# kaiidams/Kokoro-Align

Hardware: AMD Instinct MI355X
Metric: aligned audio-frames/sec (whole node), 50k x 5k lattice (higher is better)
Workload: dtype f32; 1 GPU; cfg2: T=50000 x V=64 log-probs, S=5000 phonemes (L=10001), beam_size=1000, max_move=4; batch of 8192 independent lattices per GPU per step, as 4 launches of 2048 on 4 streams; lattices_per_gpu=8192, parallelism=lattice-sharded x1, kernel_form=auto, backtrace=auto, streams_per_gpu=4

## Files before the change

kokoro-align_amd/csrc/ka_wave_backtrace.hpp:

```cpp
#pragma once
#include "ka_device.hpp"

namespace ka {

constexpr int kRcMinWaves = 8;

constexpr int kBtChunk = 16;
constexpr int kBtReach = 3 * 2 * kBtChunk;
constexpr int kBtBlocks = kBtChunk / 2;
constexpr int kBtRegs = kBtChunk * kBtBlocks / 64;
constexpr int kBtGroupsPerReg = 16 / kBtBlocks;
static_assert(16 * kBtBlocks >= kBtReach + 31, "window too narrow for the prefetch distance");

__device__ __forceinline__ int bt_window(int p_entry)
{
    const int lo = p_entry - kBtReach;
    return (lo > 0 ? lo : 0) >> 4;
}
__device__ __forceinline__ uint32_t bt_lane_offset(int w0, int lane)
{
    const int j = lane % kBtBlocks, fr = (lane / kBtBlocks) & 3, g = lane / (4 * kBtBlocks);
    return (uint32_t)g * 1024u + (uint32_t)((w0 + j) & 63) * 16u + (uint32_t)fr * 4u;
}
__device__ __forceinline__ void bt_load_guarded(uint32_t (&r)[kBtRegs], const char *chunk_base, int n, int w0, int lane)
{
    const int fr = (lane / kBtBlocks) & 3, g = lane / (4 * kBtBlocks);
    const uint32_t voff = bt_lane_offset(w0, lane);
#pragma unroll
    for (int v = 0; v < kBtRegs; ++v) {
        const int f = 4 * (v * kBtGroupsPerReg + g) + fr;
        r[v] = f < n ? *(gcu32_t)(chunk_base + (size_t)v * kBtGroupsPerReg * 1024 + voff) : 0u;
    }
}
__device__ __forceinline__ void bt_load_async(uint32_t (&r)[kBtRegs], const char *chunk_base , int w0, int lane)
{
    const uint32_t voff = bt_lane_offset(w0, lane);
#pragma unroll
    for (int v = 0; v < kBtRegs; ++v)
        asm volatile("global_load_dword %0, %1, %2" : "=&v"(r[v]) : "v"(voff), "s"(chunk_base + (size_t)v * kBtGroupsPerReg * 1024) : "memory");
}
template <int N>
__device__ __forceinline__ void bt_wait(uint32_t (&r)[2])
{
    asm volatile("s_waitcnt vmcnt(%2)" : "+v"(r[0]), "+v"(r[1]) : "i"(N) : "memory");
}
template <bool FULL>
__device__ __forceinline__ void bt_walk(const uint32_t (&r)[kBtRegs], int n, int w0, int &p, int &pathv)
{
    int q = p - 16 * w0;
    const int base = 16 * w0;
    uint32_t rr[kBtRegs];
#pragma unroll
    for (int i = 0; i < kBtRegs; ++i) rr[i] = blank_to_uniform(r[i]);
#pragma unroll
    for (int f = kBtChunk - 1; f >= 0; --f) {
        if (FULL || f < n) {
            const int grp = f >> 2;
            const int lane_base = ((grp % kBtGroupsPerReg) * 4 + (f & 3)) * kBtBlocks;
            const uint32_t w = (uint32_t)__builtin_amdgcn_readlane((int)rr[grp / kBtGroupsPerReg], (q >> 4) | lane_base);
            asm("v_writelane_b32 %0, %1, %2" : "+v"(pathv) : "s"(q), "i"(f));
            q -= bp_decode(w >> ((q * 2) & 31));
        }
    }
    pathv += base;
    p = q + base;
}

__global__ __launch_bounds__(64) void backtrace_w16_kernel(const Lattice *__restrict__ lats, const int32_t *meta, int only_flagged)
{
    const Lattice &d = lats[blockIdx.x];
    const int lane = threadIdx.x;
    if (only_flagged && !(__builtin_amdgcn_readfirstlane(meta[4 * (size_t)d.idx + 2]) & kFlagExact)) return;
    int p = __builtin_amdgcn_readfirstlane(meta[4 * (size_t)d.idx + 1]);
    if (p < 0) return;
    const char *bp = reinterpret_cast<const char *>(d.bp);
    gi32_t path = (gi32_t)d.path;
    const int T = __builtin_amdgcn_readfirstlane(d.T);
    uint32_t cur[kBtRegs], nxt[kBtRegs];
    int t0 = ((T - 1) / kBtChunk) * kBtChunk;
    int w = bt_window(p + 3 * kBtChunk);
    {
        const int n = T - t0;
        bt_load_guarded(cur, bp + (size_t)t0 * 256, n, w, lane);
        const int t1 = t0 > 0 ? t0 - kBtChunk : 0;
        const int wn = bt_window(p);
        bt_load_async(nxt, bp + (size_t)t1 * 256, wn, lane);
        int pathv = 0;
        bt_walk<false>(cur, n, w, p, pathv);
        if (lane < n) path[t0 + lane] = pathv;
        bt_wait<1>(nxt);
#pragma unroll
        for (int i = 0; i < kBtRegs; ++i) cur[i] = nxt[i];
        w = wn;
    }
    while (t0 > 0) {
        t0 -= kBtChunk;
        const int t1 = t0 > 0 ? t0 - kBtChunk : 0;
        const int wn = bt_window(p);
        bt_load_async(nxt, bp + (size_t)t1 * 256, wn, lane);
        int pathv = 0;
        bt_walk<true>(cur, kBtChunk, w, p, pathv);
        if (lane < kBtChunk) path[t0 + lane] = pathv;
        bt_wait<1>(nxt);
#pragma unroll
        for (int i = 0; i < kBtRegs; ++i) cur[i] = nxt[i];
        w = wn;
    }
}

__device__ __forceinline__ uint32_t rc_blank_to_uniform(uint32_t x)
{
    const uint32_t h = (x >> 3) & 0x11111111u, l = (x >> 2) & 0x11111111u;
    return (x & 0x33333333u) | ((h | l) << 3) | (h << 2);
}
__device__ __forceinline__ uint64_t lane_field(uint32_t count, uint32_t first)
{
    uint64_t m;
    asm("s_bfm_b64 %0, %1, %2" : "=s"(m) : "s"(count), "s"(first));
    return m;
}
#define KA_RC_E0_OUT "=&s"
#define KA_RC_E0_IN "s"
#define KA_RC_GATHER "ds_bpermute_b32 %[eln], %[lab4], %[rown]\n\tv_readfirstlane_b32 %[e0n], %[rown]\n\t"
#define KA_RC_HEAD                                                                        \
    KA_RC_GATHER                                                                          \
    "v_add_f32 %[t2], %[e0], %[sl]\n\t"                                                   \
    "v_add_f32_dpp %[t4], %[sl], %[el] wave_ror:1 row_mask:0xf bank_mask:0xf\n\t"         \
    "v_add_f32_dpp %[t5], %[sb], %[el] wave_ror:1 row_mask:0xf bank_mask:0xf\n\t"         \
    "v_add_f32 %[t0], %[e0], %[sb]\n\t"                                                   \
    "v_add_f32 %[t3], %[sb], %[el]\n\t"                                                   \
    "v_add_f32 %[t7], %[sl], %[el]\n\t"                                                   \
    "v_mov_b32_dpp %[t1], %[t2] wave_ror:1 row_mask:0xf bank_mask:0xf\n\t"                \
    "v_max_f32 %[t6], %[t7], %[t3]\n\t"
#define KA_RC_VETO "v_min_f32 %[t4], %[t4], %[veto]\n\t"
#define KA_RC_MAX                                                                         \
    "v_max3_f32 %[sl], %[t6], %[t4], %[t5]\n\t"                                           \
    "s_nop 0\n\t"                                                                         \
    "v_mov_b32_dpp %[t2], %[t1] wave_ror:1 row_mask:0xf bank_mask:0xf\n\t"                \
    "v_max3_f32 %[sb], %[t0], %[t1], %[t2]\n\t"
#define KA_RC_COMBINE                                                                     \
    "s_or_b64 %[sx], %[sa], %[sb2]\n\t"                                                   \
    "v_addc_co_u32 %[w], %[sy], %[w], %[w], %[sx]\n\t"                                    \
    "s_andn2_b64 %[sc], %[sc], %[sb2]\n\t"                                                \
    "s_or_b64 %[sc], %[sc], %[sa]\n\t"                                                    \
    "v_addc_co_u32 %[w], %[sy], %[w], %[w], %[sc]\n\t"
#define KA_RC_CODES                                                                       \
    "v_cmp_eq_f32 %[sa], %[t0], %[sb]\n\t"                                                \
    "v_addc_co_u32 %[w], %[sy], %[w], %[w], %[sa]\n\t"                                    \
    "v_cmp_eq_f32 %[sa], %[t1], %[sb]\n\t"                                                \
    "v_addc_co_u32 %[w], %[sy], %[w], %[w], %[sa]\n\t"                                    \
    "v_cmp_eq_f32 %[sa], %[t7], %[sl]\n\t"                                                \
    "v_cmp_eq_f32 %[sb2], %[t3], %[sl]\n\t"                                               \
    "v_cmp_eq_f32 %[sc], %[t4], %[sl]\n\t"                                                \
    KA_RC_COMBINE
#define KA_RC_BAND                                                                        \
    "s_bitcmp1_b32 %[open], 0\n\t"                                                        \
    "s_cbranch_scc1 .Lka_rc_open_%=\n\t"                                                  \
    "v_cndmask_b32 %[sb], %[ninf], %[sb], %[mb]\n\t"                                      \
    "v_cndmask_b32 %[sl], %[ninf], %[sl], %[ml]\n"                                        \
    ".Lka_rc_open_%=:\n\t"                                                                \
    "s_waitcnt lgkmcnt(0)"
#define KA_RC_OUTS                                                                                                              \
    [sb] "+v"(sb), [sl] "+v"(sl), [w] "+v"(word), [eln] "=&v"(el_next), [e0n] KA_RC_E0_OUT(e0_next), [t0] "=&v"(t0), [t1] "=&v"(t1),   \
    [t2] "=&v"(t2), [t3] "=&v"(t3), [t4] "=&v"(t4), [t5] "=&v"(t5), [t6] "=&v"(t6), [t7] "=&v"(t7), [sa] "=&s"(sa),             \
    [sb2] "=&s"(sb2), [sc] "=&s"(sc), [sx] "=&s"(sx), [sy] "=&s"(sy)
#define KA_RC_INS                                                                                                               \
    [e0] KA_RC_E0_IN(e0), [el] "v"(el), [rown] "v"(row_next), [lab4] "v"(lab4), [zero] "v"(zero), [open] "s"(open), [mb] "s"(mask_b),   \
    [ml] "s"(mask_l), [ninf] "v"(NINF)
template <bool ZL>
__device__ __forceinline__ void rc_frame4(float &sb, float &sl, uint32_t &word, float e0, float el, float &e0_next, float &el_next,
                                          float row_next, int lab4, int zero, float veto, uint32_t open, uint64_t mask_b,
                                          uint64_t mask_l, float NINF)
{
    float t0, t1, t2, t3, t4, t5, t6, t7;
    uint64_t sa, sb2, sc, sx, sy;
    if constexpr (ZL)
        asm volatile(KA_RC_HEAD KA_RC_VETO KA_RC_MAX KA_RC_CODES KA_RC_BAND : KA_RC_OUTS : KA_RC_INS, [veto] "v"(veto) : "memory", "scc");
    else
        asm volatile(KA_RC_HEAD KA_RC_MAX KA_RC_CODES KA_RC_BAND : KA_RC_OUTS : KA_RC_INS : "memory", "scc");
}
#undef KA_RC_HEAD
#undef KA_RC_GATHER
#undef KA_RC_E0_OUT
#undef KA_RC_E0_IN
#undef KA_RC_VETO
#undef KA_RC_MAX
#undef KA_RC_CODES
#undef KA_RC_COMBINE
#undef KA_RC_BAND
#undef KA_RC_OUTS
#undef KA_RC_INS
constexpr int kRcLanes = 62;

template <bool FULL>
__device__ __forceinline__ void rc_walk_out(const uint32_t (&codes)[kCkFrames / 8], const float (&rows)[kCkFrames], int lab4, int n,
                                            int lane, int &qq, int &pathv, int &labv, float &scv)
{
    constexpr int G = kCkFrames / 8;
    static_assert(kCkFrames == 32, "one bit per frame in a 32-bit move mask");
    const int q_in = qq;
    int j = qq >> 1;
    uint32_t cw[G];
#pragma unroll
    for (int g = 0; g < G; ++g) cw[g] = (uint32_t)__builtin_amdgcn_readlane((int)codes[g], j);
    int cl = __builtin_amdgcn_readlane(lab4, j);
    int col = (qq & 1) ? cl >> 2 : 0;
    uint32_t par = (qq & 1) ? 0u : 2u;
    uint32_t mlo = 0, mhi = 0;
#pragma unroll
    for (int f = kCkFrames - 1; f >= 0; --f) {
        if (FULL || f < n) {
            const int sc = __builtin_amdgcn_readlane(__builtin_bit_cast(int, rows[f]), col);
            asm("v_writelane_b32 %0, %1, %2" : "+v"(scv) : "s"(sc), "i"(f));
            const uint32_t mv = (uint32_t)bp_decode(cw[f >> 3] >> (4 * (7 - (f & 7)) + par));
            if (mv != 0) {
                qq -= (int)mv;
                mlo |= (mv & 1u) << f;
                mhi |= (mv >> 1) << f;
                if (f > 0) {
                    par = (qq & 1) ? 0u : 2u;
                    if ((qq >> 1) != j) {
                        j = qq >> 1;
#pragma unroll
                        for (int g = 0; g <= (f - 1) >> 3; ++g) cw[g] = (uint32_t)__builtin_amdgcn_readlane((int)codes[g], j);
                        cl = __builtin_amdgcn_readlane(lab4, j);
                    }
                    col = (qq & 1) ? cl >> 2 : 0;
                }
            }
        }
    }
    const uint32_t above_lo = (mlo >> 1) >> (lane & 31), above_hi = (mhi >> 1) >> (lane & 31);
    pathv = q_in - (__builtin_popcount(above_lo) + 2 * __builtin_popcount(above_hi));
    const int l4 = __builtin_amdgcn_ds_bpermute((pathv >> 1) << 2, lab4);
    labv = (pathv & 1) ? l4 >> 2 : 0;
}

template <int M, bool ZL, bool PAR>
__device__ __forceinline__ void backtrace_rc_body(const Lattice *__restrict__ lats, const int32_t *meta, int n_lats)
{
    const int which = PAR ? __builtin_amdgcn_readfirstlane(lattice_of_chunk(lats, n_lats, (int64_t)blockIdx.x)) : (int)blockIdx.x;
    const Lattice &d = lats[which];
    const int lane = threadIdx.x;
    if (!PAR && __builtin_amdgcn_readfirstlane(d.par)) return;
    const int32_t *mt = meta + 4 * (size_t)d.idx;
    const int flags = __builtin_amdgcn_readfirstlane(mt[2]);
    if (flags & (kFlagExact | kFlagDeclined)) return;
    if (((flags & kFlagZeroLabel) != 0) != ZL) return;
    if (__builtin_amdgcn_readfirstlane(mt[0]) != kStatusOk) return;
    int p = __builtin_amdgcn_readfirstlane(mt[1]);
    if (p < 0) return;
    const uint32_t T = (uint32_t)__builtin_amdgcn_readfirstlane(d.T);
    const uint32_t L = (uint32_t)__builtin_amdgcn_readfirstlane(d.L);
    const uint32_t B = (uint32_t)__builtin_amdgcn_readfirstlane(d.beam);
    const uint32_t halfB = B >> 1;
    const uint32_t dq = L / T, dr = L % T;
    const float NINF = ninf();
    const char *lp = reinterpret_cast<const char *>(d.lp);
    const size_t ldb = (size_t)d.ld * 4;
    const uint32_t col_off = (lane < d.V ? (uint32_t)lane : 0u) * 4u;
    gci32_t labx = (gci32_t)d.labx;
    const char *ck = reinterpret_cast<const char *>(d.bp);
    const uint32_t ck_mask = (uint32_t)__builtin_amdgcn_readfirstlane((int)d.ck_mask);
    const size_t ck_pitch = (size_t)(uint32_t)__builtin_amdgcn_readfirstlane(d.ck_pitch);
    gi32_t path = (gi32_t)d.path;
    gi32_t lab_out = (gi32_t)d.lab_out;
    gf32_t sc_out = (gf32_t)d.sc_out;

    uint32_t t0 = ((T - 1) / kCkFrames) * kCkFrames;
    if constexpr (PAR) {
        const uint32_t c = (uint32_t)((int64_t)blockIdx.x - d.chunk0);
        t0 = c * kCkFrames;
        p = __builtin_amdgcn_readfirstlane(d.entry[c]);
    }
    const auto uni = [](uint64_t v) { return (uint32_t)__builtin_amdgcn_readfirstlane((int)(uint32_t)v); };
    uint32_t q0 = uni(((uint64_t)L * t0) / T), r0 = uni(((uint64_t)L * t0) % T);
    const uint32_t D32 = uni(((uint64_t)L * kCkFrames) / T), R32 = uni(((uint64_t)L * kCkFrames) % T);
    const float inv_T = 1.0f / (float)T;

    for (;;) {
        const int n = (int)(T - t0 < (uint32_t)kCkFrames ? T - t0 : (uint32_t)kCkFrames);
        const int wlo = __builtin_amdgcn_readfirstlane((p > 96 ? p - 96 : 0) & ~1);
        const int pb = wlo + 2 * lane;
        int lab4;
        asm volatile("global_load_dword %0, %1, %2" : "=v"(lab4) : "v"((uint32_t)lane * 4u), "s"(labx + (wlo >> 1)) : "memory");
        f32x2 ckv = {NINF, NINF};
        if (t0 != 0) {
            const uint32_t off = ((uint32_t)pb & ck_mask) * 4u;
            asm volatile("global_load_dwordx2 %0, %1, %2" : "=v"(ckv) : "v"(off), "s"(ck + ((size_t)(t0 / kCkFrames) - 1) * ck_pitch) : "memory");
        }
        float rows[kCkFrames];
        {
            const char *rp = lp + (size_t)t0 * ldb;
            if (n == kCkFrames) {
#pragma unroll
                for (int f = 0; f < kCkFrames; ++f) {
                    rows[f] = row_load(col_off, rp);
                    rp += ldb;
                }
            } else {
#pragma unroll
                for (int f = 0; f < kCkFrames; ++f) {
                    rows[f] = row_load(col_off, rp);
                    rp += (f + 1 < n) ? ldb : 0;
                }
            }
        }
        asm volatile("s_waitcnt vmcnt(%2)" : "+v"(lab4), "+v"(ckv) : "i"(kCkFrames) : "memory");
        const float veto = lab4 == 0 ? NINF : __builtin_inff();
        float sb, sl;
        if (t0 == 0) {
            sb = pb == 0 ? 0.0f : NINF;
            sl = NINF;
        } else {
            const uint32_t qm = r0 >= dr ? q0 - dq : q0 - dq - 1;
            const int32_t dl = (int32_t)qm - (int32_t)halfB;
            const uint32_t lo1 = (uint32_t)(dl > 0 ? dl : 0);
            const uint32_t hi1 = (L - lo1 < B) ? L : lo1 + B;
            sb = ((uint32_t)pb >= lo1 && (uint32_t)pb < hi1 && lane < kRcLanes) ? ckv.x : NINF;
            sl = ((uint32_t)pb + 1 >= lo1 && (uint32_t)pb + 1 < hi1 && lane < kRcLanes) ? ckv.y : NINF;
        }
        uint32_t codes[kCkFrames / 8] = {};
        const auto div_T = [&](uint32_t x) {
            uint32_t qe = (uint32_t)((float)x * inv_T);
            qe -= (qe * T > x) ? 1u : 0u;
            qe += (x - qe * T >= T) ? 1u : 0u;
            return qe;
        };
        const uint32_t qnum = r0 + (uint32_t)lane * dr;
        const uint32_t qa = q0 + (uint32_t)lane * dq + div_T(qnum);
        uint64_t mask_b = 0, mask_l = 0;
        const auto band_masks = [&](int f) {
            const uint32_t q = (uint32_t)__builtin_amdgcn_readlane((int)qa, f);
            const int32_t dl = (int32_t)q - (int32_t)halfB;
            const int32_t lo = dl > 0 ? dl : 0;
            const int32_t hi = (L - (uint32_t)lo < B) ? (int32_t)L : lo + (int32_t)B;
            int32_t x = lo - wlo, y = hi - wlo;
            x = x < 0 ? 0 : x;
            y = y < 0 ? 0 : y;
            asm("" : "+s"(x), "+s"(y));
            x = x > 2 * kRcLanes ? 2 * kRcLanes : x;
            y = y > 2 * kRcLanes ? 2 * kRcLanes : y;
            const uint32_t xb = (uint32_t)(x + 1) >> 1, yb = (uint32_t)(y + 1) >> 1, xl = (uint32_t)x >> 1, yl = (uint32_t)y >> 1;
            mask_b = lane_field(yb - xb, xb);
            mask_l = lane_field(yl - xl, xl);
        };
        if constexpr (M == 4) {
            bool open = false;
            if (t0 != 0 && n == kCkFrames) {
                const uint32_t q_last = (uint32_t)__builtin_amdgcn_readlane((int)qa, kCkFrames - 1);
                const int32_t dl_last = (int32_t)q_last - (int32_t)halfB;
                const uint32_t qm = r0 >= dr ? q0 - dq : q0 - dq - 1;
                const int32_t dl = (int32_t)qm - (int32_t)halfB;
                const uint32_t lo1 = (uint32_t)(dl > 0 ? dl : 0);
                const uint32_t hi1 = (L - lo1 < B) ? L : lo1 + B;
                open = wlo > 0 && dl_last <= wlo && (uint32_t)p < hi1;
            }
            const int zero = 0;
            float e0c, elc, e0n, eln;
            row_wait_n(rows[0], kCkFrames - 1);
            asm volatile("ds_bpermute_b32 %0, %2, %4\n\t"
                         "v_readfirstlane_b32 %1, %4\n\t"
                         "s_waitcnt lgkmcnt(0)"
                         : "=&v"(elc), "=&s"(e0c) : "v"(lab4), "v"(zero), "v"(rows[0]) : "memory");
            uint32_t moves = 0;
            const uint32_t open_bit = (uint32_t)__builtin_amdgcn_readfirstlane(open ? 1 : 0);
            if (open_bit) {
                sb = ckv.x;
                sl = ckv.y;
            } else {
                const uint32_t qb = q0 + (uint32_t)(lane + 1) * dq + div_T(qnum + dr);
                moves = (uint32_t)__builtin_amdgcn_ballot_w64(qa != qb) << 1 | 1u;
            }
            asm volatile("s_nop 1" : "+v"(sb), "+v"(sl));
#pragma unroll
            for (int f = 0; f < kCkFrames; ++f) {
                if ((moves >> f) & 1u) band_masks(f);
                if (f + 1 < kCkFrames) row_wait_n(rows[f + 1], kCkFrames - 2 - f);
                rc_frame4<ZL>(sb, sl, codes[f >> 3], e0c, elc, e0n, eln, rows[f + 1 < kCkFrames ? f + 1 : f], lab4, zero, veto,
                              open_bit, mask_b, mask_l, NINF);
                e0c = e0n;
                elc = eln;
            }
        } else {
            const uint32_t qb = q0 + (uint32_t)(lane + 1) * dq + div_T(qnum + dr);
            const uint32_t moves = (uint32_t)__builtin_amdgcn_ballot_w64(qa != qb);
#pragma unroll
            for (int f = 0; f < kCkFrames; ++f) {
                if (f == 0 || ((moves >> (f > 0 ? f - 1 : 0)) & 1u)) band_masks(f);
                row_wait_n(rows[f], kCkFrames - 1 - f);
                const float el = bperm(lab4, rows[f]);
                const float e0 = first_lane(rows[f]);
                const float L1 = wave_ror1(sl);
                const float B1 = wave_ror1(sb);
                const float L2 = wave_ror1(L1);
                uint32_t &word = codes[f >> 3];
                if ((f & 7) == 0) word = 0;
                float mb, ml;
                cell_blank<M>(sb, L1, L2, e0, mb, word);
                cell_label<M, ZL>(sl, sb, L1, B1, el, veto, ml, word);
                sb = select_by_mask(NINF, mb, mask_b);
                sl = select_by_mask(NINF, ml, mask_l);
            }
        }
#pragma unroll
        for (int g = 0; g < kCkFrames / 8; ++g) codes[g] = rc_blank_to_uniform(codes[g]);
        int pathv = 0;
        int qq = p - wlo;
        int labv = 0;
        float scv = 0.0f;
        if (n == kCkFrames)
            rc_walk_out<true>(codes, rows, lab4, n, lane, qq, pathv, labv, scv);
        else
            rc_walk_out<false>(codes, rows, lab4, n, lane, qq, pathv, labv, scv);
        if (lane < n) {
            path[t0 + lane] = pathv + wlo;
            lab_out[t0 + lane] = labv;
            sc_out[t0 + lane] = scv;
        }
        p = qq + wlo;
        if (PAR || t0 == 0) break;
        t0 -= kCkFrames;
        q0 -= D32;
        if (r0 < R32) { r0 += T; q0 -= 1; }
        r0 -= R32;
    }
}

template <int M, bool ZL, bool PAR>
__global__ __launch_bounds__(64, kRcMinWaves) void backtrace_rc_kernel(const Lattice *__restrict__ lats, const int32_t *meta, int n_lats)
{
    backtrace_rc_body<M, ZL, PAR>(lats, meta, n_lats);
}
template <int M>
__global__ __launch_bounds__(64, kRcMinWaves) void backtrace_rc_chunks_kernel(const Lattice *__restrict__ lats, const int32_t *meta, int n_lats)
{
    const Lattice &d = lats[__builtin_amdgcn_readfirstlane(lattice_of_chunk(lats, n_lats, (int64_t)blockIdx.x))];
    const int flags = __builtin_amdgcn_readfirstlane(meta[4 * (size_t)d.idx + 2]);
    if (flags & kFlagZeroLabel)
        backtrace_rc_body<M, true, true>(lats, meta, n_lats);
    else
        backtrace_rc_body<M, false, true>(lats, meta, n_lats);
}

__global__ __launch_bounds__(256) void gather_outputs_kernel(const Lattice *__restrict__ lats, const int32_t *meta, int only_flagged)
{
    const Lattice &d = lats[blockIdx.y];
    if (meta[4 * (size_t)d.idx + 1] < 0) return;
    if (only_flagged && !(meta[4 * (size_t)d.idx + 2] & kFlagExact)) return;
    const int T = d.T;
    gci32_t path = (gci32_t)d.path;
    gci32_t labx = (gci32_t)d.labx;
    gcf32_t lp = (gcf32_t)d.lp;
    const size_t ld = (size_t)d.ld;
    for (int base = blockIdx.x * 1024; base < T; base += gridDim.x * 1024) {
        int t[4], pp[4], lab[4];
        float sc[4];
#pragma unroll
        for (int i = 0; i < 4; ++i) {
            t[i] = base + i * 256 + threadIdx.x;
            pp[i] = t[i] < T ? path[t[i]] : 0;
        }
#pragma unroll
        for (int i = 0; i < 4; ++i) lab[i] = (pp[i] & 1) ? (labx[pp[i] >> 1] >> 2) : 0;
#pragma unroll
        for (int i = 0; i < 4; ++i) sc[i] = t[i] < T ? lp[(size_t)t[i] * ld + lab[i]] : 0.0f;
#pragma unroll
        for (int i = 0; i < 4; ++i) {
            if (t[i] < T) {
                ((gi32_t)d.lab_out)[t[i]] = lab[i];
                ((gf32_t)d.sc_out)[t[i]] = sc[i];
            }
        }
    }
}


__global__ __launch_bounds__(64) void backtrace_generic_kernel(const Lattice *__restrict__ lats, const int32_t *meta)
{
    const Lattice &d = lats[blockIdx.x];
    const int lane = threadIdx.x;
    int64_t p = meta[4 * (size_t)d.idx + 1];
    if (p < 0) return;
    const int64_t T = d.T, L = d.L, B = d.beam, W = d.W;
    const uint8_t *bp = reinterpret_cast<const uint8_t *>(d.bp);
    if (lane == 0) {
        for (int64_t t = T - 1; t >= 0; --t) {
            int64_t lo = (L * t) / T - B / 2;
            lo = lo < 0 ? 0 : lo;
            d.path[t] = (int32_t)p;
            p -= bp[(size_t)t * (size_t)W + (size_t)(p - lo)];
        }
    }
}


}
```

Before: 7.072 billion frames/s.

## Split recompute backtrace chunk into two-cell then one-cell-per-lane phases

The M==4 recompute backtrace now handles the first 16 frames of each 32-frame chunk with the two-cells-per-lane kernel. The last 16 frames use a narrower window of one cell per lane anchored near the entry position p, with a new inline-asm frame step and a two-bit code format. The walk-out gains a second phase that decodes these one-cell codes before the original decoding. The aim is fewer instructions per frame for the later frames, where the reachable region is narrow. The cost is a cross-lane remap at the split, extra band-mask work and more code complexity.

```diff
diff --git a/kokoro-align_amd/csrc/ka_wave_backtrace.hpp b/kokoro-align_amd/csrc/ka_wave_backtrace.hpp
--- a/kokoro-align_amd/csrc/ka_wave_backtrace.hpp
+++ b/kokoro-align_amd/csrc/ka_wave_backtrace.hpp
@@ -179,6 +179,46 @@
     else
         asm volatile(KA_RC_HEAD KA_RC_MAX KA_RC_CODES KA_RC_BAND : KA_RC_OUTS : KA_RC_INS : "memory", "scc");
 }
+constexpr int kRcSplit = 16;
+constexpr int kRc1Lanes = 61;
+constexpr int kRc1Back = 59;
+static_assert(kRc1Back >= 96 - 3 * kRcSplit, "one-cell window starts above what phase 1 and phase 2 leave exact: split too early");
+static_assert(kRc1Back + 1 <= kRc1Lanes - 1 && kRc1Lanes + 3 <= 64, "one-cell window does not reach p, or leaves no idle lanes below lane 0");
+static_assert(kRcSplit >= 1 && kRcSplit < kCkFrames, "both phases have frames");
+__device__ __forceinline__ int rc_window1(int p) { return p > kRc1Back ? (p - kRc1Back) & ~1 : 0; }
+#define KA_RC1_BLOCK                                                                      \
+    "ds_bpermute_b32 %[en], %[lab1], %[rown]\n\t"                                         \
+    "v_add_f32 %[c0], %[s], %[e]\n\t"                                                     \
+    "v_mov_b32_dpp %[r1], %[s] wave_ror:1 row_mask:0xf bank_mask:0xf\n\t"                 \
+    "v_add_f32_dpp %[c1], %[s], %[e] wave_ror:1 row_mask:0xf bank_mask:0xf\n\t"           \
+    "v_add_f32 %[ev], %[e], %[vadd]\n\t"                                                  \
+    "v_mov_b32_dpp %[r2], %[r1] wave_ror:1 row_mask:0xf bank_mask:0xf\n\t"                \
+    "v_add_f32_dpp %[c2], %[r1], %[ev] wave_ror:1 row_mask:0xf bank_mask:0xf\n\t"         \
+    "v_max3_f32 %[m], %[c0], %[c1], %[c2]\n\t"                                            \
+    "v_add_f32_dpp %[c3], %[r2], %[e] wave_ror:1 row_mask:0xf bank_mask:0xf\n\t"          \
+    "v_max_f32 %[s], %[m], %[c3]\n\t"                                                     \
+    "v_cmp_eq_f32 %[sa], %[c0], %[s]\n\t"                                                 \
+    "v_cmp_eq_f32 %[sb2], %[c1], %[s]\n\t"                                                \
+    "v_cmp_eq_f32 %[sc], %[c2], %[s]\n\t"                                                 \
+    KA_RC_COMBINE                                                                         \
+    "s_bitcmp1_b32 %[open], 0\n\t"                                                        \
+    "s_cbranch_scc1 .Lka_rc1_open_%=\n\t"                                                 \
+    "v_cndmask_b32 %[s], %[ninf], %[s], %[mk]\n"                                          \
+    ".Lka_rc1_open_%=:\n\t"                                                               \
+    "s_waitcnt lgkmcnt(0)"
+__device__ __forceinline__ void rc_frame1(float &s, uint32_t &word, float e, float &e_next, float row_next, int lab1, float vadd,
+                                          uint32_t open, uint64_t mask, float NINF)
+{
+    float c0, c1, c2, c3, r1, r2, ev, m;
+    uint64_t sa, sb2, sc, sx, sy;
+    asm volatile(KA_RC1_BLOCK
+                 : [s] "+v"(s), [w] "+v"(word), [en] "=&v"(e_next), [c0] "=&v"(c0), [c1] "=&v"(c1), [c2] "=&v"(c2), [c3] "=&v"(c3),
+                   [r1] "=&v"(r1), [r2] "=&v"(r2), [ev] "=&v"(ev), [m] "=&v"(m), [sa] "=&s"(sa), [sb2] "=&s"(sb2), [sc] "=&s"(sc),
+                   [sx] "=&s"(sx), [sy] "=&s"(sy)
+                 : [e] "v"(e), [rown] "v"(row_next), [lab1] "v"(lab1), [vadd] "v"(vadd), [open] "s"(open), [mk] "s"(mask), [ninf] "v"(NINF)
+                 : "memory", "scc");
+}
+#undef KA_RC1_BLOCK
 #undef KA_RC_HEAD
 #undef KA_RC_GATHER
 #undef KA_RC_E0_OUT
@@ -192,13 +232,45 @@
 #undef KA_RC_INS
 constexpr int kRcLanes = 62;
 
-template <bool FULL>
-__device__ __forceinline__ void rc_walk_out(const uint32_t (&codes)[kCkFrames / 8], const float (&rows)[kCkFrames], int lab4, int n,
-                                            int lane, int &qq, int &pathv, int &labv, float &scv)
-{
-    constexpr int G = kCkFrames / 8;
+template <bool FULL, int SPLIT>
+__device__ __forceinline__ void rc_walk_out(const uint32_t (&codes)[kCkFrames / 8], const uint32_t (&codes2)[2], const float (&rows)[kCkFrames],
+                                            int lab4, int lab1, int d2, int n, int lane, int &qq, int &pathv, int &labv, float &scv)
+{
+    constexpr int G = (SPLIT + 7) / 8;
+    constexpr int G2 = (kCkFrames - SPLIT + 15) / 16;
     static_assert(kCkFrames == 32, "one bit per frame in a 32-bit move mask");
+    static_assert(G2 <= 2, "two words of second-phase codes at the most");
     const int q_in = qq;
+    uint32_t mlo = 0, mhi = 0;
+    if constexpr (SPLIT < kCkFrames) {
+        if (FULL || n > SPLIT) {
+            int l2 = qq - d2;
+            uint32_t cw2[G2 > 0 ? G2 : 1];
+#pragma unroll
+            for (int g = 0; g < G2; ++g) cw2[g] = (uint32_t)__builtin_amdgcn_readlane((int)codes2[g], l2);
+            int col2 = __builtin_amdgcn_readlane(lab1, l2) >> 2;
+#pragma unroll
+            for (int f = kCkFrames - 1; f >= SPLIT; --f) {
+                if (FULL || f < n) {
+                    const int k = f - SPLIT;
+                    const int sc = __builtin_amdgcn_readlane(__builtin_bit_cast(int, rows[f]), col2);
+                    asm("v_writelane_b32 %0, %1, %2" : "+v"(scv) : "s"(sc), "i"(f));
+                    const uint32_t mv = (uint32_t)bp_decode(cw2[k >> 4] >> (2 * (15 - (k & 15))));
+                    if (mv != 0) {
+                        qq -= (int)mv;
+                        mlo |= (mv & 1u) << f;
+                        mhi |= (mv >> 1) << f;
+                        if (k > 0) {
+                            l2 = qq - d2;
+#pragma unroll
+                            for (int g = 0; g <= (k - 1) >> 4; ++g) cw2[g] = (uint32_t)__builtin_amdgcn_readlane((int)codes2[g], l2);
+                            col2 = __builtin_amdgcn_readlane(lab1, l2) >> 2;
+                        }
+                    }
+                }
+            }
+        }
+    }
     int j = qq >> 1;
     uint32_t cw[G];
 #pragma unroll
@@ -206,9 +278,8 @@
     int cl = __builtin_amdgcn_readlane(lab4, j);
     int col = (qq & 1) ? cl >> 2 : 0;
     uint32_t par = (qq & 1) ? 0u : 2u;
-    uint32_t mlo = 0, mhi = 0;
-#pragma unroll
-    for (int f = kCkFrames - 1; f >= 0; --f) {
+#pragma unroll
+    for (int f = SPLIT - 1; f >= 0; --f) {
         if (FULL || f < n) {
             const int sc = __builtin_amdgcn_readlane(__builtin_bit_cast(int, rows[f]), col);
             asm("v_writelane_b32 %0, %1, %2" : "+v"(scv) : "s"(sc), "i"(f));
@@ -321,6 +392,10 @@
             sl = ((uint32_t)pb + 1 >= lo1 && (uint32_t)pb + 1 < hi1 && lane < kRcLanes) ? ckv.y : NINF;
         }
         uint32_t codes[kCkFrames / 8] = {};
+        constexpr int SPLIT = M == 4 ? kRcSplit : kCkFrames;
+        uint32_t codes2[2] = {};
+        const int w2 = __builtin_amdgcn_readfirstlane(rc_window1(p));
+        int lab1 = 0;
         const auto div_T = [&](uint32_t x) {
             uint32_t qe = (uint32_t)((float)x * inv_T);
             qe -= (qe * T > x) ? 1u : 0u;
@@ -345,6 +420,20 @@
             mask_b = lane_field(yb - xb, xb);
             mask_l = lane_field(yl - xl, xl);
         };
+        uint64_t mask_1 = 0;
+        const auto band_mask1 = [&](int f) {
+            const uint32_t q = (uint32_t)__builtin_amdgcn_readlane((int)qa, f);
+            const int32_t dl = (int32_t)q - (int32_t)halfB;
+            const int32_t lo = dl > 0 ? dl : 0;
+            const int32_t hi = (L - (uint32_t)lo < B) ? (int32_t)L : lo + (int32_t)B;
+            int32_t x = lo - w2, y = hi - w2;
+            x = x < 0 ? 0 : x;
+            y = y < 0 ? 0 : y;
+            asm("" : "+s"(x), "+s"(y));
+            x = x > kRc1Lanes ? kRc1Lanes : x;
+            y = y > kRc1Lanes ? kRc1Lanes : y;
+            mask_1 = lane_field((uint32_t)(y - x), (uint32_t)x);
+        };
         if constexpr (M == 4) {
             bool open = false;
             if (t0 != 0 && n == kCkFrames) {
@@ -370,18 +459,40 @@
                 sl = ckv.y;
             } else {
                 const uint32_t qb = q0 + (uint32_t)(lane + 1) * dq + div_T(qnum + dr);
-                moves = (uint32_t)__builtin_amdgcn_ballot_w64(qa != qb) << 1 | 1u;
+                moves = (uint32_t)__builtin_amdgcn_ballot_w64(qa != qb) << 1 | 1u | (1u << kRcSplit);
             }
             asm volatile("s_nop 1" : "+v"(sb), "+v"(sl));
+            float s1 = NINF, vadd = NINF, e1c = NINF, e1n;
 #pragma unroll
             for (int f = 0; f < kCkFrames; ++f) {
-                if ((moves >> f) & 1u) band_masks(f);
+                if (f < kRcSplit) {
+                    if ((moves >> f) & 1u) band_masks(f);
+                    if (f + 1 < kCkFrames) row_wait_n(rows[f + 1], kCkFrames - 2 - f);
+                    rc_frame4<ZL>(sb, sl, codes[f >> 3], e0c, elc, e0n, eln, rows[f + 1 < kCkFrames ? f + 1 : f], lab4, zero, veto,
+                                  open_bit, mask_b, mask_l, NINF);
+                    e0c = e0n;
+                    elc = eln;
+                    continue;
+                }
+                if (f == kRcSplit) {
+                    const int src4 = ((lane + (w2 - wlo)) >> 1) << 2;
+                    const bool odd = (lane & 1) != 0;
+                    const float xb = bperm(src4, sb), xl = bperm(src4, sl);
+                    const int l4 = __builtin_amdgcn_ds_bpermute(src4, lab4);
+                    s1 = lane < kRc1Lanes ? (odd ? xl : xb) : NINF;
+                    lab1 = odd ? l4 : 0;
+                    vadd = (!odd || (ZL && l4 == 0)) ? NINF : -0.0f;
+                    asm volatile("ds_bpermute_b32 %0, %1, %2\n\t"
+                                 "s_waitcnt lgkmcnt(0)"
+                                 : "=&v"(e1c) : "v"(lab1), "v"(rows[kRcSplit]), "v"(s1) : "memory");
+                }
+                if ((moves >> f) & 1u) band_mask1(f);
                 if (f + 1 < kCkFrames) row_wait_n(rows[f + 1], kCkFrames - 2 - f);
-                rc_frame4<ZL>(sb, sl, codes[f >> 3], e0c, elc, e0n, eln, rows[f + 1 < kCkFrames ? f + 1 : f], lab4, zero, veto,
-                              open_bit, mask_b, mask_l, NINF);
-                e0c = e0n;
-                elc = eln;
-            }
+                rc_frame1(s1, codes2[(f - kRcSplit) >> 4], e1c, e1n, rows[f + 1 < kCkFrames ? f + 1 : f], lab1, vadd, open_bit, mask_1, NINF);
+                e1c = e1n;
+            }
+            if constexpr (kRcSplit % 8 != 0) codes[kRcSplit / 8] <<= 4 * (8 - kRcSplit % 8);
+            if constexpr ((kCkFrames - kRcSplit) % 16 != 0) codes2[(kCkFrames - kRcSplit) / 16] <<= 2 * (16 - (kCkFrames - kRcSplit) % 16);
         } else {
             const uint32_t qb = q0 + (uint32_t)(lane + 1) * dq + div_T(qnum + dr);
             const uint32_t moves = (uint32_t)__builtin_amdgcn_ballot_w64(qa != qb);
@@ -404,15 +515,15 @@
             }
         }
 #pragma unroll
-        for (int g = 0; g < kCkFrames / 8; ++g) codes[g] = rc_blank_to_uniform(codes[g]);
+        for (int g = 0; g < (SPLIT + 7) / 8; ++g) codes[g] = rc_blank_to_uniform(codes[g]);
         int pathv = 0;
         int qq = p - wlo;
         int labv = 0;
         float scv = 0.0f;
         if (n == kCkFrames)
-            rc_walk_out<true>(codes, rows, lab4, n, lane, qq, pathv, labv, scv);
+            rc_walk_out<true, SPLIT>(codes, codes2, rows, lab4, lab1, w2 - wlo, n, lane, qq, pathv, labv, scv);
         else
-            rc_walk_out<false>(codes, rows, lab4, n, lane, qq, pathv, labv, scv);
+            rc_walk_out<false, SPLIT>(codes, codes2, rows, lab4, lab1, w2 - wlo, n, lane, qq, pathv, labv, scv);
         if (lane < n) {
             path[t0 + lane] = pathv + wlo;
             lab_out[t0 + lane] = labv;
```

Result: faster. 7.183 billion frames/s, median of 6 (+1.6%).
